# yahoo/bftkv

Measured on NVIDIA H100. Metric: rsa2048_signature_verifies_per_sec, higher is better.
Workload: dtype u32 limbs / u64 products (integer)

## Files before the change

### bftkv_b200/csrc/bftq.cu

```cuda
#include "../../include/bftq.h"
#include "rsa_verify.cuh"
#include "rsa_verify_r32.cuh"
#include "tally.cuh"
#include "lagrange.cuh"
#include "modexp.cuh"
#include "ed25519_fast.cuh"
#include "p256.cuh"
#include "dsa_verify.cuh"
#include "pgp_digest.cuh"
#include "pgp_parse.cuh"
#include "msg_parse.cuh"
#include "msg_decrypt.cuh"
#include "pgp_host.hpp"
#include "wotqs_host.hpp"

#include <algorithm>
#include <array>
#include <atomic>
#include <cstdio>
#include <cstdlib>
#include <cstring>
#include <chrono>
#include <condition_variable>
#include <deque>
#include <functional>
#include <map>
#include <tuple>
#include <memory>
#include <thread>
#include <mutex>
#include <string>
#include <vector>

#include <sched.h>
#include <unistd.h>

namespace {

thread_local std::string g_last_error;

int fail(int code, const std::string& msg) {
  g_last_error = msg;
  return code;
}
#define CU(call)                                                                              \
  do {                                                                                        \
    cudaError_t _e = (call);                                                                  \
    if (_e != cudaSuccess)                                                                    \
      return fail(BFTQ_ERR_CUDA, std::string(#call) + ": " + cudaGetErrorString(_e));         \
  } while (0)

constexpr int kHL = 64;
struct UBig { uint64_t w[kHL]; };

bool ge(const UBig& a, const UBig& b) {
  for (int i = kHL - 1; i >= 0; i--) { if (a.w[i] != b.w[i]) return a.w[i] > b.w[i]; }
  return true;
}
void sub(UBig& a, const UBig& b) {
  unsigned __int128 br = 0;
  for (int i = 0; i < kHL; i++) {
    unsigned __int128 d = (unsigned __int128)a.w[i] - b.w[i] - (uint64_t)br;
    a.w[i] = (uint64_t)d;
    br = (d >> 64) & 1;
  }
}
void dbl_mod(UBig& a, const UBig& n) {
  uint64_t top = a.w[kHL - 1] >> 63;
  for (int i = kHL - 1; i > 0; i--) a.w[i] = (a.w[i] << 1) | (a.w[i - 1] >> 63);
  a.w[0] <<= 1;
  if (top || ge(a, n)) sub(a, n);
}
int bitlen(const UBig& a) {
  for (int i = kHL - 1; i >= 0; i--) if (a.w[i]) return 64 * i + 64 - __builtin_clzll(a.w[i]);
  return 0;
}
void from_be(UBig& a, const uint8_t* be, size_t len) {
  memset(&a, 0, sizeof(a));
  for (size_t i = 0; i < len; i++) {
    const size_t bi = len - 1 - i;
    a.w[bi >> 3] |= (uint64_t)be[i] << (8 * (bi & 7));
  }
}
void to_digits(const UBig& a, uint32_t* d, int nd) {
  for (int i = 0; i < nd; i++) {
    int o = 28 * i;
    uint32_t v = 0;
    if (o < 64 * kHL) {
      int wi = o >> 6, sh = o & 63;
      unsigned __int128 t = a.w[wi];
      if (wi + 1 < kHL) t |= (unsigned __int128)a.w[wi + 1] << 64;
      v = (uint32_t)(t >> sh) & bftq::kDigitMask;
    }
    d[i] = v;
  }
}

struct StagingSlot {
  cudaStream_t stream = nullptr;
  uint8_t* h_pinned = nullptr;  size_t h_cap = 0;
  uint8_t* d_buf = nullptr;     size_t d_cap = 0;
  cudaEvent_t done = nullptr;
  bool busy = false;
};

}

struct PackerPool {
  struct Job {
    std::function<void()> body;
    std::function<bool()> has_work;
    unsigned max_joiners = 0, joined = 0;
    unsigned active = 0;
  };
  std::mutex mu;
  std::condition_variable cv_jobs, cv_idle;
  std::deque<std::shared_ptr<Job>> jobs;
  std::vector<std::thread> threads;
  bool stop = false;
  std::function<void()> on_start;

  void ensure(unsigned n) {
    while (threads.size() < n) threads.emplace_back([this] { loop(); });
  }
  void loop() {
    if (on_start) on_start();
    std::unique_lock<std::mutex> l(mu);
    for (;;) {
      std::shared_ptr<Job> j;
      cv_jobs.wait(l, [&] {
        if (stop) return true;
        for (auto& c : jobs) if (c->joined < c->max_joiners && c->has_work()) { j = c; return true; }
        return false;
      });
      if (stop) return;
      j->joined++; j->active++;
      l.unlock();
      j->body();
      l.lock();
      j->active--;
      cv_idle.notify_all();
    }
  }
  void run(unsigned helpers, std::function<void()> body, std::function<bool()> has_work) {
    auto j = std::make_shared<Job>();
    j->body = body; j->has_work = std::move(has_work); j->max_joiners = helpers;
    if (helpers) {
      std::lock_guard<std::mutex> l(mu);
      ensure(helpers);
      jobs.push_back(j);
    }
    if (helpers) cv_jobs.notify_all();
    body();
    if (!helpers) return;
    std::unique_lock<std::mutex> l(mu);
    for (auto it = jobs.begin(); it != jobs.end(); ++it) if (*it == j) { jobs.erase(it); break; }
    cv_idle.wait(l, [&] { return j->active == 0; });
  }
  ~PackerPool() {
    { std::lock_guard<std::mutex> l(mu); stop = true; }
    cv_jobs.notify_all();
    for (auto& t : threads) t.join();
  }
};

struct EdCache {
// ... 473 lines not shown
  return BFTQ_OK;
}
int bftq_bind_thread(bftq_engine* e) {
  if (!e) return fail(BFTQ_ERR_INVALID_ARG, "NULL argument");
  numa_bind_this_thread(e);
  return e->numa_valid ? e->numa_node : -1;
}

void bftq_shutdown(bftq_engine* e) {
  if (!e) return;
  cudaSetDevice(e->device);
  {
    std::lock_guard<std::mutex> g(e->kr_mu);
    for (bftq_keyring* kr : e->keyrings) { priv_release(kr); keyring_detach(kr); }
    e->keyrings.clear();
  }
  for (auto& kv : e->host_allocs) cudaFreeHost(kv.first);
  for (auto* s : e->slots) {
    if (s->stream) { cudaStreamSynchronize(s->stream); cudaStreamDestroy(s->stream); }
    if (s->done) cudaEventDestroy(s->done);
    if (s->h_pinned) cudaFreeHost(s->h_pinned);
    if (s->d_buf) cudaFree(s->d_buf);
    delete s;
  }
  if (e->d_keys) cudaFree(e->d_keys);
  if (e->d_keys32) cudaFree(e->d_keys32);
  cudaDeviceSynchronize();
  for (auto& b : e->scratch.free_list) cudaFree(b.first);
  for (cudaEvent_t ev : e->ed.pending) cudaEventDestroy(ev);
  if (e->ed.d_tab) cudaFree(e->ed.d_tab);
  if (e->ed.d_tabB) cudaFree(e->ed.d_tabB);
  if (e->ed.d_hdr) cudaFree(e->ed.d_hdr);
  for (void* p : e->retired) cudaFree(p);
  delete e;
}

int bftq_device_sm_count(bftq_engine* e) { return e ? e->sm_count : BFTQ_ERR_INVALID_ARG; }
int bftq_engine_set_verify_flags(bftq_engine* e, uint32_t flags) {
  if (!e || (flags & ~(uint32_t)BFTQ_F_STRICT_RANGE)) return fail(BFTQ_ERR_INVALID_ARG, "unknown flag");
  std::lock_guard<std::mutex> g(e->mu);
  e->packer_flags = flags;
  return BFTQ_OK;
}
int bftq_key_count(bftq_engine* e) {
  if (!e) return BFTQ_ERR_INVALID_ARG;
  std::lock_guard<std::mutex> g(e->mu);
  return (int)e->n_dev_keys;
}

int bftq_register_rsa_keys(bftq_engine* e, const uint8_t* n_be, const uint32_t* exps, uint32_t count,
                           uint32_t* first_index) {
  return bftq_register_rsa_keys_k(e, n_be, 256, exps, count, first_index);
}

}
namespace {
int make_key_consts(const uint8_t* n_be, uint32_t stride, uint32_t exp, bftq::RsaKeyDev& kd, bftq::r32::RsaKey32& k32, bool* is2048) {
  UBig n;
  from_be(n, n_be, stride);
  const int nb = bitlen(n);
  const int kb = (nb + 7) / 8;
  const int cls = bftq::class_of(kb);
  if (!cls || !(n.w[0] & 1)) return fail(BFTQ_ERR_UNSUPPORTED_KEY, "modulus must be odd and at most 4096 bits");
  if (exp == 0) return fail(BFTQ_ERR_UNSUPPORTED_KEY, "public exponent 0");
  memset(&kd, 0, sizeof(kd));
  to_digits(n, kd.n, bftq::kMaxDigits);
  uint32_t n0 = (uint32_t)n.w[0], inv = n0;
  for (int i = 0; i < 5; i++) inv *= 2u - n0 * inv;
  kd.n0inv = (0u - inv) & bftq::kDigitMask;
  kd.e = exp;
  kd.nbits = (uint32_t)nb;
  kd.kbytes = (uint32_t)kb;
  UBig x;
  memset(&x, 0, sizeof(x));
  x.w[0] = 1;
  int exp2 = 0;
  for (int layout = 0; layout < bftq::kNumLayouts; layout++) {
    const int digits = bftq::class_digits(cls, layout == 1 && cls != 256 ? 0 : layout);
    const int target = 2 * 28 * digits;
    while (exp2 < target) { dbl_mod(x, n); exp2++; }
    if (exp2 == target) to_digits(x, kd.r2[layout], bftq::kMaxDigits);
  }
  memset(&k32, 0, sizeof(k32));
  for (int i = 0; i < 32; i++) { k32.n[2 * i] = (uint32_t)n.w[i]; k32.n[2 * i + 1] = (uint32_t)(n.w[i] >> 32); }
  k32.n0inv = 0u - inv;
  k32.e = exp;
  k32.nbits = (uint32_t)nb;
  if (nb == 2048) {
    UBig y;
    memset(&y, 0, sizeof(y));
    y.w[0] = 1;
    for (int ex = 0; ex < 4096; ex++) dbl_mod(y, n);
    for (int i = 0; i < 32; i++) { k32.r2[2 * i] = (uint32_t)y.w[i]; k32.r2[2 * i + 1] = (uint32_t)(y.w[i] >> 32); }
  }
  if (is2048) *is2048 = !(cls == 256 && nb != 2048);
  return BFTQ_OK;
}
}
extern "C" {

int bftq_register_rsa_keys_k(bftq_engine* e, const uint8_t* n_be, uint32_t stride, const uint32_t* exps, uint32_t count,
                             uint32_t* first_index) {
  if (!e || !n_be || !exps) return fail(BFTQ_ERR_INVALID_ARG, "NULL argument");
  if (stride == 0 || stride > 512) return fail(BFTQ_ERR_INVALID_ARG, "modulus stride must be 1..512 bytes");
  std::vector<bftq::RsaKeyDev> fresh(count);
  std::vector<bftq::r32::RsaKey32> fresh32(count);
  bool fresh_all_2048 = true;
  for (uint32_t k = 0; k < count; k++) {
    bool is2048 = true;
    const int rc = make_key_consts(n_be + (size_t)k * stride, stride, exps[k], fresh[k], fresh32[k], &is2048);
    if (rc) return fail(rc, g_last_error + " (key " + std::to_string(k) + ")");
    fresh_all_2048 = fresh_all_2048 && is2048;
  }
  std::lock_guard<std::mutex> g(e->mu);
  CU(cudaSetDevice(e->device));
  const size_t old = e->n_dev_keys, want = old + count;
  if (want > e->d_keys_cap) {
    const size_t cap = std::max<size_t>(64, want * 2);
    bftq::RsaKeyDev* nd = nullptr;
    bftq::r32::RsaKey32* nd32 = nullptr;
    if (cudaMalloc((void**)&nd, cap * sizeof(bftq::RsaKeyDev)) != cudaSuccess) return fail(BFTQ_ERR_NOMEM, "key table allocation failed");
    if (cudaMalloc((void**)&nd32, cap * sizeof(bftq::r32::RsaKey32)) != cudaSuccess) { cudaFree(nd); return fail(BFTQ_ERR_NOMEM, "key table allocation failed"); }
    cudaError_t ce = cudaSuccess;
    if (old) {
      ce = cudaMemcpy(nd, e->h_keys.data(), old * sizeof(bftq::RsaKeyDev), cudaMemcpyHostToDevice);
      if (ce == cudaSuccess) ce = cudaMemcpy(nd32, e->h_keys32.data(), old * sizeof(bftq::r32::RsaKey32), cudaMemcpyHostToDevice);
    }
    if (ce == cudaSuccess && count) ce = cudaMemcpy(nd + old, fresh.data(), count * sizeof(bftq::RsaKeyDev), cudaMemcpyHostToDevice);
    if (ce == cudaSuccess && count) ce = cudaMemcpy(nd32 + old, fresh32.data(), count * sizeof(bftq::r32::RsaKey32), cudaMemcpyHostToDevice);
    if (ce != cudaSuccess) { cudaFree(nd); cudaFree(nd32); return fail(BFTQ_ERR_CUDA, std::string("key table upload: ") + cudaGetErrorString(ce)); }
    if (e->d_keys) e->retired.push_back(e->d_keys);
    if (e->d_keys32) e->retired.push_back(e->d_keys32);
    e->d_keys = nd;
    e->d_keys32 = nd32;
    e->d_keys_cap = cap;
  } else if (count) {
    CU(cudaMemcpy(e->d_keys + old, fresh.data(), count * sizeof(bftq::RsaKeyDev), cudaMemcpyHostToDevice));
    CU(cudaMemcpy(e->d_keys32 + old, fresh32.data(), count * sizeof(bftq::r32::RsaKey32), cudaMemcpyHostToDevice));
  }
  e->h_keys.insert(e->h_keys.end(), fresh.begin(), fresh.end());
  e->h_keys32.insert(e->h_keys32.end(), fresh32.begin(), fresh32.end());
  e->all_2048 = e->all_2048 && fresh_all_2048;
  e->n_dev_keys = want;
  if (first_index) *first_index = (uint32_t)old;
  return BFTQ_OK;
}

int bftq_rsa_verify_batch_dev(bftq_engine* e, const uint32_t* d_key_idx, const uint8_t* d_sig_be,
                              const uint8_t* d_digest, uint32_t hash_alg, uint64_t n_items, uint32_t flags,
                              uint8_t* d_status, void* cuda_stream) {
  return bftq_rsa_verify_batch_dev_k(e, 256, d_key_idx, d_sig_be, d_digest, hash_alg, n_items, flags, d_status, cuda_stream);
}

int bftq_rsa_verify_batch_dev_k(bftq_engine* e, uint32_t key_bytes, const uint32_t* d_key_idx, const uint8_t* d_sig_be,
                                const uint8_t* d_digest, uint32_t hash_alg, uint64_t n_items, uint32_t flags,
                                uint8_t* d_status, void* cuda_stream) {
  if (!bftq::class_supported((int)key_bytes)) return fail(BFTQ_ERR_UNSUPPORTED_KEY, "key size class not built");
  if (!e || !d_key_idx || !d_sig_be || !d_digest || !d_status) return fail(BFTQ_ERR_INVALID_ARG, "NULL argument");
  if (bftq::host_hash_dlen(hash_alg) == 0) return fail(BFTQ_ERR_INVALID_ARG, "unknown hash algorithm id");
  if (n_items == 0) return BFTQ_OK;
  CU(cudaSetDevice(e->device));
  return launch_rsa_any(e, global_keys(e), d_key_idx, d_sig_be, d_digest, hash_alg, n_items, flags, nullptr, d_status, (cudaStream_t)cuda_stream, (int)key_bytes);
}

int bftq_rsa_verify_batch(bftq_engine* e, const uint32_t* key_idx, const uint8_t* sig_be, const uint8_t* digest,
                          uint32_t hash_alg, uint64_t n_items, uint32_t flags, uint8_t* out_status) {
  return bftq_rsa_verify_batch_k(e, 256, key_idx, sig_be, digest, hash_alg, n_items, flags, out_status);
}

int bftq_rsa_verify_batch_k(bftq_engine* e, uint32_t key_bytes, const uint32_t* key_idx, const uint8_t* sig_be, const uint8_t* digest,
                            uint32_t hash_alg, uint64_t n_items, uint32_t flags, uint8_t* out_status) {
  if (!e || !key_idx || !sig_be || !digest || !out_status) return fail(BFTQ_ERR_INVALID_ARG, "NULL argument");
  if (!bftq::class_supported((int)key_bytes)) return fail(BFTQ_ERR_UNSUPPORTED_KEY, "key size class not built");
  const int dlen = bftq::host_hash_dlen(hash_alg);
  if (dlen == 0) return fail(BFTQ_ERR_INVALID_ARG, "unknown hash algorithm id");
  if (n_items == 0) return BFTQ_OK;
// ... 1009 lines not shown
```

### bftkv_b200/csrc/decrypt_host.inc

```

namespace {
namespace k6 = bftq::k6;

void wipe(void* p, size_t n) {
  volatile uint8_t* v = (volatile uint8_t*)p;
  for (size_t i = 0; i < n; i++) v[i] = 0;
}

void shl1(UBig& a) {
  for (int i = kHL - 1; i > 0; i--) a.w[i] = (a.w[i] << 1) | (a.w[i - 1] >> 63);
  a.w[0] <<= 1;
}
UBig umod(const UBig& a, const UBig& m) {
  UBig r;
  memset(&r, 0, sizeof(r));
  for (int b = bitlen(a) - 1; b >= 0; b--) {
    shl1(r);
    r.w[0] |= (a.w[b >> 6] >> (b & 63)) & 1;
    if (ge(r, m)) sub(r, m);
  }
  return r;
}
UBig umul(const UBig& a, const UBig& b) {
  UBig r;
  memset(&r, 0, sizeof(r));
  for (int i = 0; i < kHL / 2; i++) {
    unsigned __int128 c = 0;
    for (int j = 0; j < kHL / 2; j++) {
      c += (unsigned __int128)a.w[i] * b.w[j] + r.w[i + j];
      r.w[i + j] = (uint64_t)c;
      c >>= 64;
    }
    r.w[i + kHL / 2] = (uint64_t)c;
  }
  return r;
}
bool ueq(const UBig& a, const UBig& b) { return memcmp(&a, &b, sizeof(UBig)) == 0; }
void to_words(const UBig& a, uint32_t* w, int nw) {
  for (int i = 0; i < nw; i++) w[i] = (uint32_t)(a.w[i / 2] >> (32 * (i & 1)));
}
uint32_t neg_inv32(uint32_t n0) {
  uint32_t inv = n0;
  for (int i = 0; i < 5; i++) inv *= 2u - n0 * inv;
  return 0u - inv;
}
UBig shl_mod(UBig x, const UBig& m, int k) {
  for (int i = 0; i < k; i++) dbl_mod(x, m);
  return x;
}

struct SecretKey {
  uint64_t key_id = 0;
  std::vector<uint8_t> mpi[6];
  ~SecretKey() { for (auto& v : mpi) wipe(v.data(), v.size()); }
};
int parse_secret_key(const uint8_t* b, size_t n, SecretKey& k) {
  if (n < 6 || b[0] != 4) return BFTQ_ERR_UNSUPPORTED_KEY;
  if (!(b[5] == 1 || b[5] == 2 || b[5] == 3)) return BFTQ_ERR_UNSUPPORTED_KEY;
  size_t p = 6;
  for (int i = 0; i < 2; i++) {
    const uint8_t* md; size_t ml; unsigned bits;
    if (pg::read_mpi(b, n, p, md, ml, bits)) return BFTQ_ERR_MALFORMED;
    pg::strip_assign(k.mpi[i], md, ml);
  }
  pg::PubKey pk;
  if (pg::parse_public_key(b, p, pk) != pg::kOk) return BFTQ_ERR_MALFORMED;
  k.key_id = pk.key_id;
  if (p >= n) return BFTQ_ERR_MALFORMED;
  if (b[p] != 0) return BFTQ_ERR_UNSUPPORTED_KEY;
  p++;
  const size_t start = p;
  for (int i = 2; i < 6; i++) {
    const uint8_t* md; size_t ml; unsigned bits;
    if (pg::read_mpi(b, n, p, md, ml, bits)) return BFTQ_ERR_MALFORMED;
    pg::strip_assign(k.mpi[i], md, ml);
  }
  if (p + 2 > n) return BFTQ_ERR_MALFORMED;
  uint32_t sum = 0;
  for (size_t i = start; i < p; i++) sum += b[i];
  if ((sum & 0xffff) != (((uint32_t)b[p] << 8) | b[p + 1])) return BFTQ_ERR_MALFORMED;
  return BFTQ_OK;
}

int make_priv(const SecretKey& sk, k6::RsaPriv32& kp) {
  UBig n, d, p, q, u;
  from_be(n, sk.mpi[0].data(), sk.mpi[0].size());
  if (sk.mpi[2].size() > 256 || sk.mpi[3].size() > 128 || sk.mpi[4].size() > 128 || sk.mpi[5].size() > 256 || sk.mpi[0].size() > 256)
    return BFTQ_ERR_UNSUPPORTED_KEY;
  from_be(d, sk.mpi[2].data(), sk.mpi[2].size());
  from_be(p, sk.mpi[3].data(), sk.mpi[3].size());
  from_be(q, sk.mpi[4].data(), sk.mpi[4].size());
  from_be(u, sk.mpi[5].data(), sk.mpi[5].size());
  int rc = BFTQ_OK;
  if (bitlen(n) != 2048 || bitlen(p) != 1024 || bitlen(q) != 1024 || !(p.w[0] & 1) || !(q.w[0] & 1) || !ueq(umul(p, q), n)) rc = BFTQ_ERR_UNSUPPORTED_KEY;
  if (rc == BFTQ_OK) {
    memset(&kp, 0, sizeof(kp));
    UBig pm1 = p, qm1 = q, one;
    memset(&one, 0, sizeof(one)); one.w[0] = 1;
    sub(pm1, one); sub(qm1, one);
    UBig dp = umod(d, pm1), dq = umod(d, qm1), uu = umod(u, q), r2p = shl_mod(umod(one, p), p, 2048), r2q = shl_mod(umod(one, q), q, 2048);
    UBig uq = shl_mod(uu, q, 1024), pn = shl_mod(p, n, 2048);
    to_words(p, kp.p, 32); to_words(q, kp.q, 32); to_words(dp, kp.dp, 32); to_words(dq, kp.dq, 32);
    to_words(r2p, kp.r2p, 32); to_words(r2q, kp.r2q, 32); to_words(uq, kp.uq, 32); to_words(n, kp.n, 64); to_words(pn, kp.pn, 64);
    kp.p0inv = neg_inv32(kp.p[0]); kp.q0inv = neg_inv32(kp.q[0]); kp.n0inv = neg_inv32(kp.n[0]);
    wipe(&pm1, sizeof(UBig)); wipe(&qm1, sizeof(UBig)); wipe(&dp, sizeof(UBig)); wipe(&dq, sizeof(UBig)); wipe(&uu, sizeof(UBig));
    wipe(&r2p, sizeof(UBig)); wipe(&r2q, sizeof(UBig)); wipe(&uq, sizeof(UBig)); wipe(&pn, sizeof(UBig));
  }
  wipe(&d, sizeof(UBig)); wipe(&p, sizeof(UBig)); wipe(&q, sizeof(UBig)); wipe(&u, sizeof(UBig));
  return rc;
}

int run_k6a(bftq_engine* e, const k6::RsaPriv32* d_slots, const std::vector<uint32_t>& slot, const std::vector<uint8_t>& c_be,
            std::vector<uint32_t>& info, uint8_t** keep_key) {
  const uint64_t n = slot.size();
  info.assign(n, 0);
  if (keep_key) *keep_key = nullptr;
  if (!n) return BFTQ_OK;
  uint32_t *d_slot = nullptr, *d_info = nullptr; uint8_t *d_c = nullptr, *d_key = nullptr;
  int rc = BFTQ_OK;
  auto cleanup = [&]() {
    if (d_key && !(keep_key && rc == BFTQ_OK)) { cudaMemset(d_key, 0, n * 32); cudaDeviceSynchronize(); cudaFree(d_key); }
    cudaFree(d_slot); cudaFree(d_info); cudaFree(d_c);
  };
  if (cudaMalloc(&d_slot, n * 4) || cudaMalloc(&d_info, n * 4) || cudaMalloc(&d_c, n * 256) || cudaMalloc(&d_key, n * 32)) {
    cudaGetLastError(); rc = fail(BFTQ_ERR_NOMEM, "device allocation for the session-key stage failed"); cleanup(); return rc;
  }
  constexpr int kBlock = 64;
  cudaMemcpy(d_slot, slot.data(), n * 4, cudaMemcpyHostToDevice);
  cudaMemcpy(d_c, c_be.data(), n * 256, cudaMemcpyHostToDevice);
  const uint64_t blocks = std::min<uint64_t>((n + kBlock / 4 - 1) / (kBlock / 4), (uint64_t)std::max(1, e->sm_count) * 16);
  k6::rsa_crt_decrypt_kernel<kBlock><<<(unsigned)blocks, kBlock>>>(d_slots, d_slot, d_c, n, d_info, d_key);
// ... 363 lines not shown
```

### bftkv_b200/csrc/rsa_verify_r32.cuh

```cuda
#pragma once
#include <cstdint>
#include <cuda_runtime.h>
#include "rsa_verify.cuh"

namespace bftq {
namespace r32 {

constexpr int T = 4;

#define BFTQ_CHAIN8_BODY(first)                                                              \
  first " %0, %18, %26, %0;  madc.hi.cc.u32 %1, %18, %26, %1;"                                \
  "madc.lo.cc.u32 %2, %19, %26, %2;  madc.hi.cc.u32 %3, %19, %26, %3;"                        \
  "madc.lo.cc.u32 %4, %20, %26, %4;  madc.hi.cc.u32 %5, %20, %26, %5;"                        \
  "madc.lo.cc.u32 %6, %21, %26, %6;  madc.hi.cc.u32 %7, %21, %26, %7;"                        \
  "madc.lo.cc.u32 %8, %22, %26, %8;  madc.hi.cc.u32 %9, %22, %26, %9;"                        \
  "madc.lo.cc.u32 %10, %23, %26, %10; madc.hi.cc.u32 %11, %23, %26, %11;"                     \
  "madc.lo.cc.u32 %12, %24, %26, %12; madc.hi.cc.u32 %13, %24, %26, %13;"                     \
  "madc.lo.cc.u32 %14, %25, %26, %14; madc.hi.cc.u32 %15, %25, %26, %15;"                     \
  "addc.cc.u32 %16, %16, 0; addc.u32 %17, %17, 0;"
#define BFTQ_CHAIN8_OPS(p, c0, c1, x)                                                                                     \
  : "+r"(p[0]), "+r"(p[1]), "+r"(p[2]), "+r"(p[3]), "+r"(p[4]), "+r"(p[5]), "+r"(p[6]), "+r"(p[7]), "+r"(p[8]), "+r"(p[9]), \
    "+r"(p[10]), "+r"(p[11]), "+r"(p[12]), "+r"(p[13]), "+r"(p[14]), "+r"(p[15]), "+r"(c0), "+r"(c1)                      \
  : "r"(x[0]), "r"(x[2]), "r"(x[4]), "r"(x[6]), "r"(x[8]), "r"(x[10]), "r"(x[12]), "r"(x[14]), "r"(m)

// ... 57 lines not shown
template <int W>
__device__ __forceinline__ uint32_t ripple_add(uint32_t (&v)[W], const uint32_t x) {
  uint32_t c;
  asm volatile("add.cc.u32 %0, %0, %1;" : "+r"(v[0]) : "r"(x));
#pragma unroll
  for (int k = 1; k < W; k++) asm volatile("addc.cc.u32 %0, %0, 0;" : "+r"(v[k]));
  asm volatile("addc.u32 %0, 0, 0;" : "=r"(c));
  return c;
}
template <int W>
__device__ __forceinline__ uint32_t ripple_sub(uint32_t (&v)[W], const uint32_t x) {
  uint32_t b;
  asm volatile("sub.cc.u32 %0, %0, %1;" : "+r"(v[0]) : "r"(x));
#pragma unroll
  for (int k = 1; k < W; k++) asm volatile("subc.cc.u32 %0, %0, 0;" : "+r"(v[k]));
  asm volatile("subc.u32 %0, 0, 0;" : "=r"(b));
  return b & 1u;
}
template <int W>
__device__ __forceinline__ uint32_t sub_n(uint32_t (&d)[W], const uint32_t (&v)[W], const uint32_t (&n)[W]) {
  uint32_t b;
  asm volatile("sub.cc.u32 %0, %1, %2;" : "=r"(d[0]) : "r"(v[0]), "r"(n[0]));
#pragma unroll
  for (int k = 1; k < W; k++) asm volatile("subc.cc.u32 %0, %1, %2;" : "=r"(d[k]) : "r"(v[k]), "r"(n[k]));
  asm volatile("subc.u32 %0, 0, 0;" : "=r"(b));
  return b & 1u;
}

__device__ __forceinline__ uint32_t lane_carry_in(const uint32_t gbits, const uint32_t pbits, const int r, uint32_t& out) {
  const uint32_t c1 = gbits & 1u;
  const uint32_t c2 = ((gbits >> 1) & 1u) | (((pbits >> 1) & 1u) & c1);
  const uint32_t c3 = ((gbits >> 2) & 1u) | (((pbits >> 2) & 1u) & c2);
  out = ((gbits >> 3) & 1u) | (((pbits >> 3) & 1u) & c3);
  return r == 0 ? 0u : (r == 1 ? c1 : (r == 2 ? c2 : c3));
}

template <int W, bool CT = false>
__device__ __forceinline__ void mont_finish(uint32_t (&out)[W], Acc<W>& A, const uint32_t cin, const uint32_t Z, const uint32_t (&n)[W],
                                            const int r, const int gbase) {
  uint32_t v[W], hi;
  asm volatile("add.cc.u32 %0, %1, %2;" : "=r"(v[0]) : "r"(A.E[0]), "r"(Z));
#pragma unroll
  for (int k = 1; k < W; k++) asm volatile("addc.cc.u32 %0, %1, %2;" : "=r"(v[k]) : "r"(A.E[k]), "r"(A.O[k - 1]));
  asm volatile("addc.u32 %0, %1, %2;" : "=r"(hi) : "r"(A.E[W]), "r"(A.O[W - 1]));
  uint32_t from_below = __shfl_up_sync(kFull, hi, 1, T);
  if (r == 0) from_below = 0u;
  const uint32_t g = ripple_add(v, from_below + cin);
  bool ones = true;
#pragma unroll
  for (int k = 0; k < W; k++) ones = ones && (v[k] == 0xffffffffu);
  const uint32_t gb = __ballot_sync(kFull, g != 0u) >> gbase;
  const uint32_t pb = __ballot_sync(kFull, ones) >> gbase;
  uint32_t ctop;
  const uint32_t ci = lane_carry_in(gb, pb, r, ctop);
  ripple_add(v, ci);
  const uint32_t top_hi = __shfl_sync(kFull, hi, gbase + T - 1);
  const bool overflow = (top_hi + ctop) != 0u;
  if (CT || __any_sync(kFull, overflow)) {
    uint32_t d[W];
    const uint32_t bo = sub_n(d, v, n);
    bool zeros = true;
#pragma unroll
    for (int k = 0; k < W; k++) zeros = zeros && (d[k] == 0u);
    const uint32_t bgb = __ballot_sync(kFull, bo != 0u) >> gbase;
    const uint32_t bpb = __ballot_sync(kFull, zeros) >> gbase;
    uint32_t btop;
    const uint32_t bi = lane_carry_in(bgb, bpb, r, btop);
    ripple_sub(d, bi);
    if (CT) {
      const uint32_t m = 0u - (uint32_t)overflow;
#pragma unroll
      for (int k = 0; k < W; k++) v[k] = (d[k] & m) | (v[k] & ~m);
    } else if (overflow) {
#pragma unroll
      for (int k = 0; k < W; k++) v[k] = d[k];
    }
  }
#pragma unroll
  for (int k = 0; k < W; k++) out[k] = v[k];
}

template <int W, bool STEP_SYNC = false, bool CT = false>
__device__ __forceinline__ void mont_mul(uint32_t (&out)[W], const uint32_t (&a)[W], const uint32_t (&b)[W],
                                         const uint32_t (&n)[W], const uint32_t n0inv, const int r, const int gbase) {
  Acc<W> A;
#pragma unroll
  for (int k = 0; k < W + 4; k++) A.E[k] = 0u;
#pragma unroll
  for (int k = 0; k < W + 2; k++) A.O[k] = 0u;
  uint32_t cin = 0u;
  uint32_t Z = 0u;
#ifndef BFTQ_MUL_UNROLL
#define BFTQ_MUL_UNROLL 1
#endif
  constexpr int kMulUnroll = BFTQ_MUL_UNROLL;
#pragma unroll kMulUnroll
  for (int owner = 0; owner < T; owner++) {
    if (STEP_SYNC) __syncthreads();
    const int src = gbase + owner;
#pragma unroll
    for (int jj = 0; jj < W; jj += 2) {
      const uint32_t b0 = __shfl_sync(kFull, b[jj], src);
      const uint32_t b1 = __shfl_sync(kFull, b[jj + 1], src);
      mac_off0_even(A, a, b0, cin);
      uint32_t q0 = (A.E[0] + Z) * n0inv;
      q0 = __shfl_sync(kFull, q0, gbase);
      mac_off0_odd(A, a, b0);
      mac_off1_even(A, a, b1);
      mac_off1_odd(A, a, b1);
      mac_off0_even_nocin(A, n, q0);
      mac_off0_odd(A, n, q0);
      const uint64_t s0 = (uint64_t)A.E[0] + Z;
      const uint32_t p0 = (uint32_t)s0, c0 = (uint32_t)(s0 >> 32);
      uint32_t q1 = (A.E[1] + A.O[0] + c0) * n0inv;
      q1 = __shfl_sync(kFull, q1, gbase);
      mac_off1_even(A, n, q1);
      mac_off1_odd(A, n, q1);
      const uint64_t s1 = (uint64_t)A.E[1] + A.O[0] + c0;
      const uint32_t p1 = (uint32_t)s1;
      cin = (uint32_t)(s1 >> 32);
      Z = A.O[1];
      uint32_t r0 = __shfl_down_sync(kFull, p0, 1, T);
      uint32_t r1 = __shfl_down_sync(kFull, p1, 1, T);
      if (r == T - 1) { r0 = 0u; r1 = 0u; }
#pragma unroll
      for (int k = 0; k < W + 2; k++) A.E[k] = A.E[k + 2];
      A.E[W + 2] = 0u; A.E[W + 3] = 0u;
#pragma unroll
      for (int k = 0; k < W; k++) A.O[k] = A.O[k + 2];
      A.O[W] = 0u; A.O[W + 1] = 0u;
      asm volatile("add.cc.u32 %0, %0, %4; addc.cc.u32 %1, %1, %5; addc.cc.u32 %2, %2, 0; addc.u32 %3, %3, 0;"
                   : "+r"(A.E[W - 2]), "+r"(A.E[W - 1]), "+r"(A.E[W]), "+r"(A.E[W + 1]) : "r"(r0), "r"(r1));
    }
  }
  mont_finish<W, CT>(out, A, cin, Z, n, r, gbase);
}

template <int W>
__device__ __forceinline__ bool group_ge(const uint32_t (&x)[W], const uint32_t (&n)[W], const int gbase) {
  bool gt = false, lt = false;
#pragma unroll
  for (int j = W - 1; j >= 0; j--) {
    if (!gt && !lt) { gt = x[j] > n[j]; lt = x[j] < n[j]; }
  }
  const uint32_t gmask = ((1u << T) - 1u) << gbase;
  const uint32_t gtb = __ballot_sync(kFull, gt) & gmask;
  const uint32_t ltb = __ballot_sync(kFull, lt) & gmask;
  return gtb >= ltb;
}

template <int W>
__device__ __forceinline__ void cond_sub(uint32_t (&x)[W], const uint32_t (&n)[W], const int r, const int gbase) {
  const bool ge = group_ge(x, n, gbase);
  uint32_t d[W];
  const uint32_t bo = sub_n(d, x, n);
  bool zeros = true;
#pragma unroll
  for (int k = 0; k < W; k++) zeros = zeros && (d[k] == 0u);
  const uint32_t bgb = __ballot_sync(kFull, bo != 0u) >> gbase;
  const uint32_t bpb = __ballot_sync(kFull, zeros) >> gbase;
  uint32_t btop;
  const uint32_t bi = lane_carry_in(bgb, bpb, r, btop);
  ripple_sub(d, bi);
  if (ge) {
#pragma unroll
    for (int k = 0; k < W; k++) x[k] = d[k];
  }
}

}
}
#include "rsa_square_r32.cuh"
namespace bftq {
namespace r32 {

struct RsaKey32 {
  uint32_t n[64];
  uint32_t r2[64];
  uint32_t n0inv;
  uint32_t e;
  uint32_t nbits;
  uint32_t pad;
};

#ifndef BFTQ_K1_SYNC
#define BFTQ_K1_SYNC 2
#endif
#ifndef BFTQ_K1_UNIFIED
#define BFTQ_K1_UNIFIED 1
#endif
template <int BLOCK, int MIN_BLOCKS, bool SQ>
__global__ void __launch_bounds__(BLOCK, MIN_BLOCKS)
rsa_verify_r32_kernel(const RsaKey32* __restrict__ keys, const uint32_t nkeys, const uint32_t* __restrict__ key_idx,
                      const uint8_t* __restrict__ sig, const uint8_t* __restrict__ digest, const uint32_t hash_alg,
                      const uint64_t n_items, const uint32_t flags, const uint8_t* __restrict__ pre_status,
                      uint8_t* __restrict__ status) {
  constexpr int W = 16;
  constexpr int kGroupsPerWarp = 32 / T;
  __shared__ uint32_t xm_s[W][BLOCK];
  __shared__ int nbmax_s;
  constexpr bool kStepSync = BFTQ_K1_SYNC >= 3;
  const int lane = threadIdx.x & 31;
  const int r = lane & (T - 1);
  const int gbase = lane & ~(T - 1);
  const int plen = c_hash_prefix[hash_alg].len;
  const int dlen = c_hash_prefix[hash_alg].dlen;
  const uint64_t warp_global = (uint64_t)blockIdx.x * (BLOCK / 32) + (threadIdx.x >> 5);
  const uint64_t warps_total = (uint64_t)gridDim.x * (BLOCK / 32);
  const uint32_t gmask = ((1u << T) - 1u) << gbase;

  for (uint64_t bbase = (uint64_t)blockIdx.x * (BLOCK / 32) * kGroupsPerWarp; bbase < n_items; bbase += warps_total * kGroupsPerWarp) {
    const uint64_t wbase = bbase + (uint64_t)(threadIdx.x >> 5) * kGroupsPerWarp;
    if (BFTQ_K1_SYNC >= 1) __syncthreads();
    const uint64_t item_raw = wbase + (uint64_t)(lane / T);
    const bool valid = item_raw < n_items;
    const uint64_t item = valid ? item_raw : (n_items - 1);
    uint32_t kidx = __ldg(key_idx + item);
    const bool known = kidx < nkeys;
    if (!known) kidx = 0u;
    const RsaKey32* __restrict__ key = keys + kidx;

    uint32_t nd[W], y[W], t[W];
#pragma unroll
    for (int j = 0; j < W; j++) nd[j] = __ldg(&key->n[r * W + j]);
    const uint32_t n0inv = __ldg(&key->n0inv);
    const uint32_t e = __ldg(&key->e);
    const uint8_t* sp = sig + item * (uint64_t)kRsaBytes;
    bool s_ge_n;
#pragma unroll
    for (int j = 0; j < W; j++) y[j] = be_word(sp, r * W + j);
    s_ge_n = group_ge(y, nd, gbase);
    const int nb = 32 - __clz(e);
    int nbmax = nb;
#pragma unroll
    for (int o = 16; o >= 1; o >>= 1) nbmax = max(nbmax, __shfl_xor_sync(kFull, nbmax, o));
    if (BFTQ_K1_SYNC >= 2) {
      if (threadIdx.x == 0) nbmax_s = 0;
      __syncthreads();
      if (lane == 0) atomicMax(&nbmax_s, nbmax);
      __syncthreads();
      nbmax = nbmax_s;
    }
#if BFTQ_K1_UNIFIED
    int op = 0, bit = nbmax - 2;
#pragma unroll 1
    for (;;) {
      if (op == 1) {
        if (SQ) mont_sqr<kStepSync>(t, y, nd, n0inv, r, gbase); else mont_mul<W, kStepSync>(t, y, y, nd, n0inv, r, gbase);
        if (BFTQ_K1_SYNC >= 2) __syncthreads();
        if (bit <= nb - 2) {
#pragma unroll
          for (int j = 0; j < W; j++) y[j] = t[j];
        }
        const bool mul = bit >= 1 && bit <= nb - 2 && ((e >> bit) & 1u);
        if (__any_sync(kFull, mul)) op = 2;
        else { bit--; op = bit >= 0 ? 1 : 3; }
      } else {
        uint32_t bop[W];
        if (op == 0) {
#pragma unroll
          for (int j = 0; j < W; j++) bop[j] = __ldg(&key->r2[r * W + j]);
        } else if (op == 2) {
#pragma unroll
          for (int j = 0; j < W; j++) bop[j] = xm_s[j][threadIdx.x];
        } else {
#pragma unroll
          for (int j = 0; j < W; j++) bop[j] = ((e & 1u) && nb >= 2) ? be_word(sp, r * W + j) : ((r == 0 && j == 0) ? 1u : 0u);
        }
        mont_mul(t, y, bop, nd, n0inv, r, gbase);
        if (op == 3) break;
        if (op == 0) {
#pragma unroll
          for (int j = 0; j < W; j++) { y[j] = t[j]; xm_s[j][threadIdx.x] = t[j]; }
          op = bit >= 0 ? 1 : 3;
        } else {
          if (bit <= nb - 2 && ((e >> bit) & 1u)) {
#pragma unroll
            for (int j = 0; j < W; j++) y[j] = t[j];
          }
          bit--;
          op = bit >= 0 ? 1 : 3;
        }
      }
    }
#else
    {
      uint32_t r2[W];
#pragma unroll
      for (int j = 0; j < W; j++) r2[j] = __ldg(&key->r2[r * W + j]);
      mont_mul(t, y, r2, nd, n0inv, r, gbase);
#pragma unroll
      for (int j = 0; j < W; j++) y[j] = t[j];
    }
#pragma unroll
    for (int j = 0; j < W; j++) xm_s[j][threadIdx.x] = y[j];
#pragma unroll 1
    for (int bit = nbmax - 2; bit >= 1; bit--) {
      const bool active = bit <= nb - 2;
      if (SQ) mont_sqr<kStepSync>(t, y, nd, n0inv, r, gbase); else mont_mul<W, kStepSync>(t, y, y, nd, n0inv, r, gbase);
      if (BFTQ_K1_SYNC >= 2) __syncthreads();
      if (active) {
#pragma unroll
        for (int j = 0; j < W; j++) y[j] = t[j];
      }
      const bool mul = active && ((e >> bit) & 1u);
      if (__any_sync(kFull, mul)) {
        uint32_t xm[W];
#pragma unroll
        for (int j = 0; j < W; j++) xm[j] = xm_s[j][threadIdx.x];
        mont_mul(t, y, xm, nd, n0inv, r, gbase);
        if (mul) {
#pragma unroll
          for (int j = 0; j < W; j++) y[j] = t[j];
        }
      }
    }
    if (__any_sync(kFull, nb >= 2)) {
      if (SQ) mont_sqr(t, y, nd, n0inv, r, gbase); else mont_mul(t, y, y, nd, n0inv, r, gbase);
      if (nb >= 2) {
#pragma unroll
        for (int j = 0; j < W; j++) y[j] = t[j];
      }
    }
    {
      uint32_t m1[W];
#pragma unroll
      for (int j = 0; j < W; j++) m1[j] = ((e & 1u) && nb >= 2) ? be_word(sp, r * W + j) : ((r == 0 && j == 0) ? 1u : 0u);
      mont_mul(t, y, m1, nd, n0inv, r, gbase);
    }
#endif
    cond_sub(t, nd, r, gbase);

    const uint8_t* dp = digest + item * (uint64_t)dlen;
    bool eq = true;
#pragma unroll
    for (int j = 0; j < W; j++) eq = eq && (em_word(r * W + j, dp, plen, dlen, hash_alg) == t[j]);
    const uint32_t eqb = __ballot_sync(kFull, eq) & gmask;
    if (valid && r == 0) {
      uint8_t st = (eqb == gmask) ? (uint8_t)0 : (uint8_t)1;
      if ((flags & 1u) && s_ge_n) st = 1;
      if (__ldg(&key->nbits) != 2048u) st = 1;
      if (!known) st = 4;
      if (pre_status != nullptr) {
        const uint8_t pre = __ldg(pre_status + item_raw);
        if (pre != 0) st = pre;
      }
      status[item_raw] = st;
    }
  }
}

}
}
```

Measured before the change: 54.88 million.

## Verify RSA signatures in Montgomery domain with precomputed per-key constants, skipping conversions

The kernel no longer converts the signature into Montgomery form with an R^2 multiply and no longer converts the result back out. It runs the exponentiation on the raw signature and folds the leftover R factors into per-key constants (c16/c32, hc16/hc32) computed on the host. The encoded-message check is a partial Montgomery multiply that uses only 1 or 2 owner limb groups, since the padding is mostly constant, followed by group subtractions and a comparison against 0 or n. This drops the entry multiply and shortens the final one, at the cost of a more intricate equality check, extra host precomputation and larger per-key constant storage.

```diff
diff --git a/bftkv_b200/csrc/bftq.cu b/bftkv_b200/csrc/bftq.cu
--- a/bftkv_b200/csrc/bftq.cu
+++ b/bftkv_b200/csrc/bftq.cu
@@ -13,6 +13,7 @@
 #include "msg_decrypt.cuh"
 #include "pgp_host.hpp"
 #include "wotqs_host.hpp"
+#include "bignum_host.hpp"
 
 #include <algorithm>
 #include <array>
@@ -50,38 +51,8 @@
       return fail(BFTQ_ERR_CUDA, std::string(#call) + ": " + cudaGetErrorString(_e));         \
   } while (0)
 
-constexpr int kHL = 64;
-struct UBig { uint64_t w[kHL]; };
-
-bool ge(const UBig& a, const UBig& b) {
-  for (int i = kHL - 1; i >= 0; i--) { if (a.w[i] != b.w[i]) return a.w[i] > b.w[i]; }
-  return true;
-}
-void sub(UBig& a, const UBig& b) {
-  unsigned __int128 br = 0;
-  for (int i = 0; i < kHL; i++) {
-    unsigned __int128 d = (unsigned __int128)a.w[i] - b.w[i] - (uint64_t)br;
-    a.w[i] = (uint64_t)d;
-    br = (d >> 64) & 1;
-  }
-}
-void dbl_mod(UBig& a, const UBig& n) {
-  uint64_t top = a.w[kHL - 1] >> 63;
-  for (int i = kHL - 1; i > 0; i--) a.w[i] = (a.w[i] << 1) | (a.w[i - 1] >> 63);
-  a.w[0] <<= 1;
-  if (top || ge(a, n)) sub(a, n);
-}
-int bitlen(const UBig& a) {
-  for (int i = kHL - 1; i >= 0; i--) if (a.w[i]) return 64 * i + 64 - __builtin_clzll(a.w[i]);
-  return 0;
-}
-void from_be(UBig& a, const uint8_t* be, size_t len) {
-  memset(&a, 0, sizeof(a));
-  for (size_t i = 0; i < len; i++) {
-    const size_t bi = len - 1 - i;
-    a.w[bi >> 3] |= (uint64_t)be[i] << (8 * (bi & 7));
-  }
-}
+using namespace bftq::hostbig;
+
 void to_digits(const UBig& a, uint32_t* d, int nd) {
   for (int i = 0; i < nd; i++) {
     int o = 28 * i;
@@ -721,16 +692,16 @@
     if (exp2 == target) to_digits(x, kd.r2[layout], bftq::kMaxDigits);
   }
   memset(&k32, 0, sizeof(k32));
-  for (int i = 0; i < 32; i++) { k32.n[2 * i] = (uint32_t)n.w[i]; k32.n[2 * i + 1] = (uint32_t)(n.w[i] >> 32); }
+  to_words(n, k32.n, 64);
   k32.n0inv = 0u - inv;
   k32.e = exp;
   k32.nbits = (uint32_t)nb;
   if (nb == 2048) {
-    UBig y;
-    memset(&y, 0, sizeof(y));
-    y.w[0] = 1;
-    for (int ex = 0; ex < 4096; ex++) dbl_mod(y, n);
-    for (int i = 0; i < 32; i++) { k32.r2[2 * i] = (uint32_t)y.w[i]; k32.r2[2 * i + 1] = (uint32_t)(y.w[i] >> 32); }
+    const bftq::hostbig::VerifyConsts vc = bftq::hostbig::verify_consts(n, exp);
+    to_words(vc.c16, k32.c16, 64);
+    to_words(vc.hc16, k32.hc16, 64);
+    to_words(vc.c32, k32.c32, 64);
+    to_words(vc.hc32, k32.hc32, 64);
   }
   if (is2048) *is2048 = !(cls == 256 && nb != 2048);
   return BFTQ_OK;
diff --git a/bftkv_b200/csrc/bignum_host.hpp b/bftkv_b200/csrc/bignum_host.hpp
--- /dev/null
+++ b/bftkv_b200/csrc/bignum_host.hpp
@@ -0,0 +1,112 @@
+#pragma once
+#include <cstddef>
+#include <cstdint>
+#include <cstring>
+
+namespace bftq {
+namespace hostbig {
+
+constexpr int kHL = 64;
+struct UBig { uint64_t w[kHL]; };
+
+inline bool ge(const UBig& a, const UBig& b) {
+  for (int i = kHL - 1; i >= 0; i--) { if (a.w[i] != b.w[i]) return a.w[i] > b.w[i]; }
+  return true;
+}
+inline void sub(UBig& a, const UBig& b) {
+  unsigned __int128 br = 0;
+  for (int i = 0; i < kHL; i++) {
+    unsigned __int128 d = (unsigned __int128)a.w[i] - b.w[i] - (uint64_t)br;
+    a.w[i] = (uint64_t)d;
+    br = (d >> 64) & 1;
+  }
+}
+inline void dbl_mod(UBig& a, const UBig& n) {
+  uint64_t top = a.w[kHL - 1] >> 63;
+  for (int i = kHL - 1; i > 0; i--) a.w[i] = (a.w[i] << 1) | (a.w[i - 1] >> 63);
+  a.w[0] <<= 1;
+  if (top || ge(a, n)) sub(a, n);
+}
+inline UBig shl_mod(UBig x, const UBig& m, int k) {
+  for (int i = 0; i < k; i++) dbl_mod(x, m);
+  return x;
+}
+inline int bitlen(const UBig& a) {
+  for (int i = kHL - 1; i >= 0; i--) if (a.w[i]) return 64 * i + 64 - __builtin_clzll(a.w[i]);
+  return 0;
+}
+inline void from_be(UBig& a, const uint8_t* be, size_t len) {
+  memset(&a, 0, sizeof(a));
+  for (size_t i = 0; i < len; i++) {
+    const size_t bi = len - 1 - i;
+    a.w[bi >> 3] |= (uint64_t)be[i] << (8 * (bi & 7));
+  }
+}
+inline void to_words(const UBig& a, uint32_t* w, int nw) {
+  for (int i = 0; i < nw; i++) w[i] = (uint32_t)(a.w[i / 2] >> (32 * (i & 1)));
+}
+
+inline UBig mont2048(const UBig& a, const UBig& b, const UBig& n, const uint64_t n0inv) {
+  constexpr int L = 32;
+  uint64_t t[L + 2] = {0};
+  for (int i = 0; i < L; i++) {
+    unsigned __int128 c = 0;
+    for (int j = 0; j < L; j++) {
+      c += (unsigned __int128)a.w[j] * b.w[i] + t[j];
+      t[j] = (uint64_t)c;
+      c >>= 64;
+    }
+    c += t[L];
+    t[L] = (uint64_t)c;
+    t[L + 1] = (uint64_t)(c >> 64);
+    const uint64_t m = t[0] * n0inv;
+    c = ((unsigned __int128)m * n.w[0] + t[0]) >> 64;
+    for (int j = 1; j < L; j++) {
+      c += (unsigned __int128)m * n.w[j] + t[j];
+      t[j - 1] = (uint64_t)c;
+      c >>= 64;
+    }
+    c += t[L];
+    t[L - 1] = (uint64_t)c;
+    t[L] = t[L + 1] + (uint64_t)(c >> 64);
+  }
+  UBig r;
+  memset(&r, 0, sizeof(r));
+  for (int j = 0; j < L; j++) r.w[j] = t[j];
+  if (t[L] || ge(r, n)) sub(r, n);
+  return r;
+}
+
+struct VerifyConsts { UBig c16, hc16, c32, hc32; };
+inline VerifyConsts verify_consts(const UBig& n, const uint32_t e) {
+  uint64_t inv = n.w[0];
+  for (int i = 0; i < 5; i++) inv *= 2u - n.w[0] * inv;
+  const uint64_t n0inv = 0u - inv;
+  UBig one;
+  memset(&one, 0, sizeof(one));
+  one.w[0] = 1;
+  UBig c = one;
+  for (int bit = 30 - __builtin_clz(e); bit >= 0; bit--) {
+    c = mont2048(c, c, n, n0inv);
+    if ((e >> bit) & 1u) c = mont2048(c, one, n, n0inv);
+  }
+  VerifyConsts k;
+  k.c16 = shl_mod(c, n, 512);
+  k.c32 = shl_mod(k.c16, n, 512);
+  const UBig cr = shl_mod(k.c32, n, 1024);
+  auto top = [](int split) {
+    UBig h, low;
+    memset(&h, 0, sizeof(h));
+    memset(&low, 0, sizeof(low));
+    h.w[2033 / 64] = 1ull << (2033 % 64);
+    low.w[split / 64] = 1;
+    sub(h, low);
+    return h;
+  };
+  k.hc16 = mont2048(top(512), cr, n, n0inv);
+  k.hc32 = mont2048(top(1024), cr, n, n0inv);
+  return k;
+}
+
+}
+}
diff --git a/bftkv_b200/csrc/decrypt_host.inc b/bftkv_b200/csrc/decrypt_host.inc
--- a/bftkv_b200/csrc/decrypt_host.inc
+++ b/bftkv_b200/csrc/decrypt_host.inc
@@ -36,17 +36,10 @@
   return r;
 }
 bool ueq(const UBig& a, const UBig& b) { return memcmp(&a, &b, sizeof(UBig)) == 0; }
-void to_words(const UBig& a, uint32_t* w, int nw) {
-  for (int i = 0; i < nw; i++) w[i] = (uint32_t)(a.w[i / 2] >> (32 * (i & 1)));
-}
 uint32_t neg_inv32(uint32_t n0) {
   uint32_t inv = n0;
   for (int i = 0; i < 5; i++) inv *= 2u - n0 * inv;
   return 0u - inv;
-}
-UBig shl_mod(UBig x, const UBig& m, int k) {
-  for (int i = 0; i < k; i++) dbl_mod(x, m);
-  return x;
 }
 
 struct SecretKey {
diff --git a/bftkv_b200/csrc/rsa_verify_r32.cuh b/bftkv_b200/csrc/rsa_verify_r32.cuh
--- a/bftkv_b200/csrc/rsa_verify_r32.cuh
+++ b/bftkv_b200/csrc/rsa_verify_r32.cuh
@@ -163,7 +163,8 @@
 
 template <int W, bool STEP_SYNC = false, bool CT = false>
 __device__ __forceinline__ void mont_mul(uint32_t (&out)[W], const uint32_t (&a)[W], const uint32_t (&b)[W],
-                                         const uint32_t (&n)[W], const uint32_t n0inv, const int r, const int gbase) {
+                                         const uint32_t (&n)[W], const uint32_t n0inv, const int r, const int gbase,
+                                         const int owners = T) {
   Acc<W> A;
 #pragma unroll
   for (int k = 0; k < W + 4; k++) A.E[k] = 0u;
@@ -177,6 +178,7 @@
   constexpr int kMulUnroll = BFTQ_MUL_UNROLL;
 #pragma unroll kMulUnroll
   for (int owner = 0; owner < T; owner++) {
+    if (owner == owners) break;
     if (STEP_SYNC) __syncthreads();
     const int src = gbase + owner;
 #pragma unroll
@@ -231,10 +233,8 @@
 }
 
 template <int W>
-__device__ __forceinline__ void cond_sub(uint32_t (&x)[W], const uint32_t (&n)[W], const int r, const int gbase) {
-  const bool ge = group_ge(x, n, gbase);
-  uint32_t d[W];
-  const uint32_t bo = sub_n(d, x, n);
+__device__ __forceinline__ uint32_t group_sub(uint32_t (&d)[W], const uint32_t (&x)[W], const uint32_t (&y)[W], const int r, const int gbase) {
+  const uint32_t bo = sub_n(d, x, y);
   bool zeros = true;
 #pragma unroll
   for (int k = 0; k < W; k++) zeros = zeros && (d[k] == 0u);
@@ -243,6 +243,14 @@
   uint32_t btop;
   const uint32_t bi = lane_carry_in(bgb, bpb, r, btop);
   ripple_sub(d, bi);
+  return btop;
+}
+
+template <int W>
+__device__ __forceinline__ void cond_sub(uint32_t (&x)[W], const uint32_t (&n)[W], const int r, const int gbase) {
+  const bool ge = group_ge(x, n, gbase);
+  uint32_t d[W];
+  group_sub(d, x, n, r, gbase);
   if (ge) {
 #pragma unroll
     for (int k = 0; k < W; k++) x[k] = d[k];
@@ -257,7 +265,10 @@
 
 struct RsaKey32 {
   uint32_t n[64];
-  uint32_t r2[64];
+  uint32_t c16[64];
+  uint32_t hc16[64];
+  uint32_t c32[64];
+  uint32_t hc32[64];
   uint32_t n0inv;
   uint32_t e;
   uint32_t nbits;
@@ -278,7 +289,7 @@
                       uint8_t* __restrict__ status) {
   constexpr int W = 16;
   constexpr int kGroupsPerWarp = 32 / T;
-  __shared__ uint32_t xm_s[W][BLOCK];
+  __shared__ uint32_t y_s[W][BLOCK];
   __shared__ int nbmax_s;
   constexpr bool kStepSync = BFTQ_K1_SYNC >= 3;
   const int lane = threadIdx.x & 31;
@@ -286,6 +297,8 @@
   const int gbase = lane & ~(T - 1);
   const int plen = c_hash_prefix[hash_alg].len;
   const int dlen = c_hash_prefix[hash_alg].dlen;
+  const bool wide = plen + dlen > 63;
+  const int check_owners = wide ? 2 : 1;
   const uint64_t warp_global = (uint64_t)blockIdx.x * (BLOCK / 32) + (threadIdx.x >> 5);
   const uint64_t warps_total = (uint64_t)gridDim.x * (BLOCK / 32);
   const uint32_t gmask = ((1u << T) - 1u) << gbase;
@@ -307,6 +320,8 @@
     const uint32_t n0inv = __ldg(&key->n0inv);
     const uint32_t e = __ldg(&key->e);
     const uint8_t* sp = sig + item * (uint64_t)kRsaBytes;
+    const uint8_t* dp = digest + item * (uint64_t)dlen;
+    const uint32_t* ck = wide ? key->c32 : key->c16;
     bool s_ge_n;
 #pragma unroll
     for (int j = 0; j < W; j++) y[j] = be_word(sp, r * W + j);
@@ -323,7 +338,7 @@
       nbmax = nbmax_s;
     }
 #if BFTQ_K1_UNIFIED
-    int op = 0, bit = nbmax - 2;
+    int bit = nbmax - 2, op = bit >= 0 ? 1 : 3;
 #pragma unroll 1
     for (;;) {
       if (op == 1) {
@@ -333,50 +348,35 @@
 #pragma unroll
           for (int j = 0; j < W; j++) y[j] = t[j];
         }
-        const bool mul = bit >= 1 && bit <= nb - 2 && ((e >> bit) & 1u);
+        const bool mul = bit <= nb - 2 && ((e >> bit) & 1u);
         if (__any_sync(kFull, mul)) op = 2;
         else { bit--; op = bit >= 0 ? 1 : 3; }
       } else {
         uint32_t bop[W];
-        if (op == 0) {
-#pragma unroll
-          for (int j = 0; j < W; j++) bop[j] = __ldg(&key->r2[r * W + j]);
-        } else if (op == 2) {
-#pragma unroll
-          for (int j = 0; j < W; j++) bop[j] = xm_s[j][threadIdx.x];
+        if (op == 3) {
+#pragma unroll 1
+          for (int j = 0; j < W; j++) y_s[j][threadIdx.x] = em_word(r * W + j, dp, plen, dlen, hash_alg);
+#pragma unroll
+          for (int j = 0; j < W; j++) { bop[j] = y_s[j][threadIdx.x]; y_s[j][threadIdx.x] = y[j]; y[j] = __ldg(&ck[r * W + j]); }
         } else {
 #pragma unroll
-          for (int j = 0; j < W; j++) bop[j] = ((e & 1u) && nb >= 2) ? be_word(sp, r * W + j) : ((r == 0 && j == 0) ? 1u : 0u);
+          for (int j = 0; j < W; j++) bop[j] = be_word(sp, r * W + j);
         }
-        mont_mul(t, y, bop, nd, n0inv, r, gbase);
+        mont_mul(t, y, bop, nd, n0inv, r, gbase, op == 2 ? T : check_owners);
         if (op == 3) break;
-        if (op == 0) {
-#pragma unroll
-          for (int j = 0; j < W; j++) { y[j] = t[j]; xm_s[j][threadIdx.x] = t[j]; }
-          op = bit >= 0 ? 1 : 3;
-        } else {
-          if (bit <= nb - 2 && ((e >> bit) & 1u)) {
-#pragma unroll
-            for (int j = 0; j < W; j++) y[j] = t[j];
-          }
-          bit--;
-          op = bit >= 0 ? 1 : 3;
+        if (bit <= nb - 2 && ((e >> bit) & 1u)) {
+#pragma unroll
+          for (int j = 0; j < W; j++) y[j] = t[j];
         }
+        bit--;
+        op = bit >= 0 ? 1 : 3;
       }
     }
+#pragma unroll
+    for (int j = 0; j < W; j++) y[j] = y_s[j][threadIdx.x];
 #else
-    {
-      uint32_t r2[W];
-#pragma unroll
-      for (int j = 0; j < W; j++) r2[j] = __ldg(&key->r2[r * W + j]);
-      mont_mul(t, y, r2, nd, n0inv, r, gbase);
-#pragma unroll
-      for (int j = 0; j < W; j++) y[j] = t[j];
-    }
-#pragma unroll
-    for (int j = 0; j < W; j++) xm_s[j][threadIdx.x] = y[j];
 #pragma unroll 1
-    for (int bit = nbmax - 2; bit >= 1; bit--) {
+    for (int bit = nbmax - 2; bit >= 0; bit--) {
       const bool active = bit <= nb - 2;
       if (SQ) mont_sqr<kStepSync>(t, y, nd, n0inv, r, gbase); else mont_mul<W, kStepSync>(t, y, y, nd, n0inv, r, gbase);
       if (BFTQ_K1_SYNC >= 2) __syncthreads();
@@ -386,36 +386,34 @@
       }
       const bool mul = active && ((e >> bit) & 1u);
       if (__any_sync(kFull, mul)) {
-        uint32_t xm[W];
-#pragma unroll
-        for (int j = 0; j < W; j++) xm[j] = xm_s[j][threadIdx.x];
-        mont_mul(t, y, xm, nd, n0inv, r, gbase);
+        uint32_t sx[W];
+#pragma unroll
+        for (int j = 0; j < W; j++) sx[j] = be_word(sp, r * W + j);
+        mont_mul(t, y, sx, nd, n0inv, r, gbase);
         if (mul) {
 #pragma unroll
           for (int j = 0; j < W; j++) y[j] = t[j];
         }
       }
     }
-    if (__any_sync(kFull, nb >= 2)) {
-      if (SQ) mont_sqr(t, y, nd, n0inv, r, gbase); else mont_mul(t, y, y, nd, n0inv, r, gbase);
-      if (nb >= 2) {
-#pragma unroll
-        for (int j = 0; j < W; j++) y[j] = t[j];
-      }
-    }
     {
-      uint32_t m1[W];
-#pragma unroll
-      for (int j = 0; j < W; j++) m1[j] = ((e & 1u) && nb >= 2) ? be_word(sp, r * W + j) : ((r == 0 && j == 0) ? 1u : 0u);
-      mont_mul(t, y, m1, nd, n0inv, r, gbase);
+      uint32_t ca[W], lb[W];
+#pragma unroll
+      for (int j = 0; j < W; j++) { ca[j] = __ldg(&ck[r * W + j]); lb[j] = em_word(r * W + j, dp, plen, dlen, hash_alg); }
+      mont_mul(t, ca, lb, nd, n0inv, r, gbase, check_owners);
     }
 #endif
+    cond_sub(y, nd, r, gbase);
     cond_sub(t, nd, r, gbase);
-
-    const uint8_t* dp = digest + item * (uint64_t)dlen;
+    uint32_t d[W];
+    const uint32_t b = group_sub(d, y, t, r, gbase);
+    const uint32_t* hk = wide ? key->hc32 : key->hc16;
+#pragma unroll
+    for (int j = 0; j < W; j++) y[j] = __ldg(&hk[r * W + j]);
+    group_sub(t, y, d, r, gbase);
     bool eq = true;
 #pragma unroll
-    for (int j = 0; j < W; j++) eq = eq && (em_word(r * W + j, dp, plen, dlen, hash_alg) == t[j]);
+    for (int j = 0; j < W; j++) eq = eq && (t[j] == (b ? nd[j] : 0u));
     const uint32_t eqb = __ballot_sync(kFull, eq) & gmask;
     if (valid && r == 0) {
       uint8_t st = (eqb == gmask) ? (uint8_t)0 : (uint8_t)1;
```

Measured after the change: 57.46 million (median of 6 runs). 4.7% higher.
